# ebanalyse/ebnerd-benchmark

Hardware: AMD Instinct MI355X
Metric: training impressions/sec (higher is better)
Workload: dtype f32

## Files before the change

### ebnerd-benchmark_amd/csrc/ebn_gemm.hip

```cpp
#include <stdlib.h>

#include "ebn_common.h"
#include "ebn_finish.h"
#include "ebn_tn_finale.h"

typedef float ebn_f32x4 __attribute__((ext_vector_type(4)));
typedef int ebn_i32x4 __attribute__((ext_vector_type(4)));
__device__ ebn_f32x4 ebn_raw_buffer_load_x4(ebn_i32x4 rsrc, int voffset, int soffset, int aux) __asm("llvm.amdgcn.raw.buffer.load.v4f32");
__device__ void ebn_raw_buffer_load_lds(ebn_i32x4 rsrc, __attribute__((address_space(3))) void* lds, int size, int voffset,
                                        int soffset, int offset, int aux) __asm("llvm.amdgcn.raw.buffer.load.lds");

int ebn_gemm_direct_tn_slices(int64_t M, int64_t N, int64_t K);
int ebn_gemm_direct_tn_launch(int64_t M, int64_t N, int64_t K, float alpha, const float* A, int64_t lda, const float* B, int64_t ldb,
                              float* part, hipStream_t s);
bool ebn_gemm_direct_wanted(int32_t transA, int32_t transB, int64_t M, int64_t N, int64_t K);
int ebn_gemm_direct_launch(int32_t transB, int64_t M, int64_t N, int64_t K, float alpha, const float* A, int64_t lda, const float* B,
                           int64_t ldb, float* C, int64_t ldc, hipStream_t s);

namespace {

typedef float f32x16 __attribute__((ext_vector_type(16)));


typedef float f32x4n __attribute__((ext_vector_type(4)));
__device__ __forceinline__ float4 gload4(const __attribute__((address_space(1))) float* p) {
  const f32x4n t = *reinterpret_cast<const __attribute__((address_space(1))) f32x4n*>(p);
  return make_float4(t.x, t.y, t.z, t.w);
}
typedef ebn_i32x4 i32x4n;
__device__ __forceinline__ i32x4n make_rsrc(const float* base) {
  const unsigned long long a = reinterpret_cast<unsigned long long>(base);
  i32x4n r;
  r.x = static_cast<int>(static_cast<uint32_t>(a));
  r.y = static_cast<int>(static_cast<uint32_t>(a >> 32) & 0xFFFFu);
  r.z = -1;
  r.w = 0x00020000;
  return r;
}
__device__ __forceinline__ float4 bload4(i32x4n r, uint32_t lane_bytes, uint32_t slab_bytes) {
  const f32x4n t = ebn_raw_buffer_load_x4(r, static_cast<int>(lane_bytes), static_cast<int>(slab_bytes), 0);
  return make_float4(t.x, t.y, t.z, t.w);
}

constexpr int GEMM_WPE = 3;
constexpr int BK = 16;
constexpr int PAD = 4;
constexpr int GEMM_THREADS = 256;

template <int BMN, bool KCONTIG, bool VEC, int PADX = PAD>
struct TileLoader {
  static constexpr int VECS = BMN * BK / 4;
  static constexpr int PER_THREAD = VECS / GEMM_THREADS;
  static_assert(VECS % GEMM_THREADS == 0, "tile/thread mismatch");

  __device__ static __forceinline__ float4 load(const float* __restrict__ P, int64_t ld, int64_t mn0,
                                                int64_t k0, int64_t MN, int64_t Kdim, int v) {
    int64_t gmn, gk;
    if (KCONTIG) {
      gmn = mn0 + v / (BK / 4);
      gk = k0 + (v % (BK / 4)) * 4;
    } else {
      gk = k0 + v / (BMN / 4);
      gmn = mn0 + (v % (BMN / 4)) * 4;
    }
    const int64_t off = KCONTIG ? (gmn * ld + gk) : (gk * ld + gmn);
    if (VEC) {
      const bool valid = (gmn < MN) && (gk < Kdim);
      const float4 r = *reinterpret_cast<const float4*>(P + (valid ? off : 0));
      float4 z;
      z.x = valid ? r.x : 0.f;
      z.y = valid ? r.y : 0.f;
      z.z = valid ? r.z : 0.f;
      z.w = valid ? r.w : 0.f;
      return z;
    }
    float4 r = make_float4(0.f, 0.f, 0.f, 0.f);
    if (KCONTIG) {
      if (gmn < MN) {
        const float* p = P + off;
        if (gk + 0 < Kdim) r.x = p[0];
        if (gk + 1 < Kdim) r.y = p[1];
        if (gk + 2 < Kdim) r.z = p[2];
        if (gk + 3 < Kdim) r.w = p[3];
      }
    } else {
      if (gk < Kdim) {
        const float* p = P + off;
        if (gmn + 0 < MN) r.x = p[0];
        if (gmn + 1 < MN) r.y = p[1];
        if (gmn + 2 < MN) r.z = p[2];
        if (gmn + 3 < MN) r.w = p[3];
      }
    }
    return r;
  }

  __device__ static __forceinline__ void store(float* __restrict__ S, int v, float4 r) {
    constexpr int LD = BMN + PADX;
    if (KCONTIG) {
      const int mn = v / (BK / 4);
      const int kq = v % (BK / 4);
      *reinterpret_cast<float4*>(&S[(mn * 4 + (kq ^ ((mn >> 2) & 3))) * 4]) = r;
    } else {
      const int k = v / (BMN / 4);
      const int mq = v % (BMN / 4);
      *reinterpret_cast<float4*>(&S[k * LD + mq * 4]) = r;
    }
  }
};

struct GemmEpi {
  const float* rs;
  const float* cv;
  int64_t ldcv;
  int32_t L;
  const float* bias;
  float* colsum = nullptr;
  const float* l2w = nullptr;
  float two_lambda = 0.f;
  const int32_t* rowmap = nullptr;
  int64_t rowmap_rows = 0;
  int32_t* oob = nullptr;
#ifdef EBN_GEMM_EXP_STAGGER
  uint32_t stagger_pct = 0;
#endif
};

template <int BM, int BN, int WAVES_M, bool TA, bool TB, bool VEC, int EPI = 0>
__global__ __launch_bounds__(GEMM_THREADS, GEMM_WPE) void gemm_f32_kernel(
    int64_t M, int64_t N, int64_t K, float alpha, const float* __restrict__ A, int64_t lda,
    const float* __restrict__ B, int64_t ldb, float beta, float* __restrict__ C, int64_t ldc,
    int64_t k_per_split, float* __restrict__ Cpart, GemmEpi epi) {
  constexpr int WAVES_N = 4 / WAVES_M;
  constexpr int WTM = BM / WAVES_M;
  constexpr int WTN = BN / WAVES_N;
  constexpr int TM = WTM / 32;
  constexpr int TN = WTN / 32;
  constexpr bool GLDS_A = VEC;
  constexpr bool GLDS_B = GLDS_A;
  constexpr int PADA = GLDS_A ? 0 : PAD, PADB = GLDS_B ? 0 : PAD;
  constexpr int LDA_S = BM + PADA;
  constexpr int LDB_S = BN + PADB;
  using LA = TileLoader<BM, !TA, VEC, PADA>;
  using LB = TileLoader<BN, TB, VEC, PADB>;

  constexpr bool A_KC = !TA, B_KC = TB;
  constexpr int A_FLOATS = A_KC ? BM * BK : BK * LDA_S, B_FLOATS = B_KC ? BN * BK : BK * LDB_S;
  __shared__ __attribute__((aligned(16))) float smem[2 * (A_FLOATS + B_FLOATS)];
#define EBN_AS(b) (smem + (b) * A_FLOATS)
#define EBN_BS(b) (smem + 2 * A_FLOATS + (b) * B_FLOATS)

  const int tid = threadIdx.x;
  const int lane = tid & 63;
  const int wave = __builtin_amdgcn_readfirstlane(tid >> 6);
  const int wm = wave / WAVES_N;
  const int wn = wave % WAVES_N;
  const int64_t GX = gridDim.x, GY = gridDim.y, GZ = gridDim.z;
  const int64_t per_z = GX * GY, nwg = per_z * GZ;
  const int64_t vb = static_cast<int64_t>(blockIdx.y) * gridDim.x + blockIdx.x + per_z * blockIdx.z;
  int64_t m0 = 0, n0 = 0, kbeg = 0, kend = 0, zsplit = 0;
  int nk = 0, nk_full = 0, nk_main = 0;
// ... 148 lines not shown
  if (VEC) {                                                                             \
    const int krem__ = static_cast<int>(kend - kbeg) - (KT) * BK;                        \
    _Pragma("unroll") for (int i = 0; i < LA::PER_THREAD; ++i) {                         \
      const int v__ = tid + i * GEMM_THREADS;                                            \
      EBN_TAIL_PIECE(ra[i], arsrc, oa[i], sa, TA ? v__ / (BM / 4) : (v__ % (BK / 4)) * 4); \
    }                                                                                    \
    _Pragma("unroll") for (int i = 0; i < LB::PER_THREAD; ++i) {                         \
      const int v__ = tid + i * GEMM_THREADS;                                            \
      EBN_TAIL_PIECE(rb[i], brsrc, ob[i], sb, TB ? (v__ % (BK / 4)) * 4 : v__ / (BN / 4)); \
    }                                                                                    \
  } else {                                                                               \
    const int64_t k0__ = kbeg + static_cast<int64_t>(KT) * BK;                           \
    _Pragma("unroll") for (int i = 0; i < LA::PER_THREAD; ++i)                           \
        ra[i] = LA::load(A, lda, m0, k0__, M, kend, tid + i * GEMM_THREADS);             \
    _Pragma("unroll") for (int i = 0; i < LB::PER_THREAD; ++i)                           \
        rb[i] = LB::load(B, ldb, n0, k0__, N, kend, tid + i * GEMM_THREADS);             \
  }                                                                                      \
  } while (0)
#define EBN_STORE_PART(BUF)                                                              \
  do {                                                                                   \
    _Pragma("unroll") for (int i = 0; i < LA::PER_THREAD; ++i) LA::store(EBN_AS(BUF), tid + i * GEMM_THREADS, ra[i]); \
    _Pragma("unroll") for (int i = 0; i < LB::PER_THREAD; ++i) LB::store(EBN_BS(BUF), tid + i * GEMM_THREADS, rb[i]); \
  } while (0)

  const int kl = lane >> 5;
  const int il = lane & 31;
  {
#pragma unroll
  for (int i = 0; i < TM; ++i)
#pragma unroll
    for (int j = 0; j < TN; ++j)
#pragma unroll
      for (int r = 0; r < 16; ++r) acc[i][j][r] = 0.f;
  if (nk_main > 0) {
    EBN_FETCH_FULL(0);
    EBN_STORE_FULL(0);
    __syncthreads();
  }
#define EBN_MMA(CUR)  \
  {  \
    const float* as = A_KC ? EBN_AS((CUR)) + (wm * WTM + il) * 16 : EBN_AS((CUR)) + (4 * kl) * LDA_S + wm * WTM + il;  \
    const float* bs = B_KC ? EBN_BS((CUR)) + (wn * WTN + il) * 16 : EBN_BS((CUR)) + (4 * kl) * LDB_S + wn * WTN + il;  \
    const int sw = (il >> 2) & 3;  \
_Pragma("unroll")  \
    for (int j8 = 0; j8 < BK / 8; ++j8) {  \
      float a[TM][4], b[TN][4];  \
_Pragma("unroll")  \
      for (int i = 0; i < TM; ++i) {  \
        if (A_KC) {  \
          const float* pa__ = as + i * 32 * 16 + (((2 * j8 + kl) ^ sw) * 4);  \
          a[i][0] = pa__[0]; a[i][1] = pa__[1]; a[i][2] = pa__[2]; a[i][3] = pa__[3];  \
        } else {  \
_Pragma("unroll")  \
          for (int w = 0; w < 4; ++w) a[i][w] = as[(8 * j8 + w) * LDA_S + i * 32];  \
        }  \
      }  \
_Pragma("unroll")  \
      for (int j = 0; j < TN; ++j) {  \
        if (B_KC) {  \
          const float* pb__ = bs + j * 32 * 16 + (((2 * j8 + kl) ^ sw) * 4);  \
          b[j][0] = pb__[0]; b[j][1] = pb__[1]; b[j][2] = pb__[2]; b[j][3] = pb__[3];  \
        } else {  \
_Pragma("unroll")  \
          for (int w = 0; w < 4; ++w) b[j][w] = bs[(8 * j8 + w) * LDB_S + j * 32];  \
        }  \
      }  \
_Pragma("unroll")  \
      for (int w = 0; w < 4; ++w)  \
_Pragma("unroll")  \
        for (int i = 0; i < TM; ++i)  \
_Pragma("unroll")  \
          for (int j = 0; j < TN; ++j)  \
            acc[i][j] = __builtin_amdgcn_mfma_f32_32x32x2f32(a[i][w], b[j][w], acc[i][j], 0, 0, 0);  \
    }  \
  }
#define EBN_SLAB(CUR, KT)  \
  {  \
    const bool next__ = (KT) + 1 < nk_main;  \
    if (next__) EBN_FETCH_FULL((CUR) ^ 1);  \
    EBN_MMA(CUR)  \
    if (next__) EBN_STORE_FULL((CUR) ^ 1);  \
    __syncthreads();  \
  }
  for (int kt = 0; kt < nk_main; kt += 2) {
    EBN_SLAB(0, kt);
    if (kt + 1 < nk_main) EBN_SLAB(1, kt + 1);
  }
#undef EBN_SLAB
  if (nk_main < nk) {
    int cur = nk_main & 1;
    EBN_FETCH_PART(nk_main);
    EBN_STORE_PART(cur);
    __syncthreads();
    for (int kt = nk_main; kt < nk; ++kt) {
      if (kt + 1 < nk) EBN_FETCH_PART(kt + 1);
      EBN_MMA(cur)
      if (kt + 1 < nk) EBN_STORE_PART(cur ^ 1);
      __syncthreads();
      cur ^= 1;
    }
  }
  const int64_t em0 = m0, en0 = n0, ezs = zsplit;

  if constexpr (EPI == 1 || EPI == 2) {
    const bool split = GZ > 1;
    float* out = split ? (Cpart + ezs * M * N) : C;
    const int64_t ldo = split ? N : ldc;
    const bool read_c = !split && beta != 0.f;
#pragma unroll
    for (int i = 0; i < TM; ++i) {
#pragma unroll
      for (int j = 0; j < TN; ++j) {
        const int64_t col = en0 + wn * WTN + j * 32 + (lane & 31);
        const bool col_ok = col < N;
        const int64_t colc = col_ok ? col : N - 1;
        const int64_t row_base = em0 + wm * WTM + i * 32 + 4 * (lane >> 5);
        float add[16];
#pragma unroll
        for (int r = 0; r < 16; ++r) add[r] = 0.f;
        if (EPI == 1 && !split) {
#pragma unroll
          for (int r = 0; r < 16; ++r) {
            const int64_t row = row_base + (r & 3) + 8 * (r >> 2);
            const uint32_t rowc = static_cast<uint32_t>(row < M ? row : M - 1);
            add[r] = epi.rs[rowc] * epi.cv[static_cast<int64_t>(rowc / static_cast<uint32_t>(epi.L)) * epi.ldcv + colc];
          }
        }
        if (EPI == 2 && !split) {
          const float bv = epi.bias[colc];
#pragma unroll
          for (int r = 0; r < 16; ++r) add[r] = bv;
        }
        if (read_c) {
#pragma unroll
          for (int r = 0; r < 16; ++r) {
            const int64_t row = row_base + (r & 3) + 8 * (r >> 2);
            add[r] = fmaf(beta, out[(row < M ? row : M - 1) * ldo + colc], add[r]);
          }
        }
#pragma unroll
        for (int r = 0; r < 16; ++r) {
          const int64_t row = row_base + (r & 3) + 8 * (r >> 2);
          float v = fmaf(alpha, acc[i][j][r], add[r]);
          if (EPI == 2 && !split) v = fmaxf(v, 0.f);
          if (col_ok && row < M) out[row * ldo + col] = v;
        }
      }
    }

  } else {
    const bool split = GZ > 1;
    float* out = split ? (Cpart + ezs * M * N) : C;
    const int64_t ldo = split ? N : ldc;
#pragma unroll
    for (int i = 0; i < TM; ++i) {
#pragma unroll
      for (int j = 0; j < TN; ++j) {
        const int64_t col = en0 + wn * WTN + j * 32 + (lane & 31);
        if (col >= N) continue;
#pragma unroll
        for (int r = 0; r < 16; ++r) {
          const int64_t row = em0 + wm * WTM + i * 32 + (r & 3) + 8 * (r >> 2) + 4 * (lane >> 5);
          if (row >= M) continue;
          float v = alpha * acc[i][j][r];
          if (!split && beta != 0.f) v += beta * out[row * ldo + col];
          if (EPI == 1 && !split)
            v = fmaf(epi.rs[row], epi.cv[static_cast<int64_t>(static_cast<uint32_t>(row) / static_cast<uint32_t>(epi.L)) * epi.ldcv + col], v);
          if (EPI == 2 && !split) v = fmaxf(v + epi.bias[col], 0.f);
#if defined(EBN_GEMM_EXP_NOSTORE)
          if (v == 1.2345e38f) out[row * ldo + col] = v;
#elif defined(EBN_GEMM_EXP_NT)
          __builtin_nontemporal_store(v, &out[row * ldo + col]);
#else
          out[row * ldo + col] = v;
#endif
        }
      }
    }

  }
  }
#undef EBN_MMA
#undef EBN_FETCH_FULL
#undef EBN_FETCH_PART
#undef EBN_STORE_FULL
#undef EBN_STORE_PART
#undef EBN_TAIL_PIECE
#undef EBN_GLDS_A_DST
#undef EBN_GLDS_B_DST
#undef EBN_AS
#undef EBN_BS
#undef EBN_STORE_SLAB
}

__global__ __launch_bounds__(256) void splitk_reduce_kernel(const float* __restrict__ part, int splits,
                                                            int64_t M, int64_t N, float beta,
                                                            float* __restrict__ C, int64_t ldc, GemmEpi epi) {
  ebn_splitk_sum_body(blockIdx.x * 256u + threadIdx.x, gridDim.x * 256u, part, splits, static_cast<uint32_t>(M * N), static_cast<uint32_t>(N),
                      beta, C, ldc, epi.rs, epi.cv, epi.ldcv, epi.L, epi.bias);
}

template <int BM, int BN, int WAVES_M>
int launch_gemm(int transA, int transB, int64_t M, int64_t N, int64_t K, float alpha, const float* A,
                int64_t lda, const float* B, int64_t ldb, float beta, float* C, int64_t ldc, int vecA,
                int vecB, int splits, int64_t k_per_split, float* part, hipStream_t s, int site, GemmEpi epi) {
  dim3 grid(static_cast<unsigned>(ebn_ceil_div(N, BN)), static_cast<unsigned>(ebn_ceil_div(M, BM)),
            static_cast<unsigned>(splits));
  dim3 block(GEMM_THREADS);
#ifdef EBN_GEMM_EXP_STAGGER
  static const uint32_t stagger_pct = getenv("EBN_GEMM_STAGGER_PCT") ? static_cast<uint32_t>(atoi(getenv("EBN_GEMM_STAGGER_PCT"))) : 0u;
  epi.stagger_pct = splits == 1 ? stagger_pct : 0u;
#endif
#define EBN_GEMM_LAUNCH(TA, TB)                                                                            \
  do {                                                                                                    \
    if (vecA && vecB)                                                                                     \
      EBN_LAUNCH((gemm_f32_kernel<BM, BN, WAVES_M, TA, TB, true>), grid, block, 0, s, M, N, K, alpha, A, lda, \
                         B, ldb, beta, C, ldc, k_per_split, part, epi);                       \
    else if constexpr (BM == 64 && BN == 64)  \
      EBN_LAUNCH((gemm_f32_kernel<BM, BN, WAVES_M, TA, TB, false>), grid, block, 0, s, M, N, K, alpha, A,  \
                         lda, B, ldb, beta, C, ldc, k_per_split, part, epi);                  \
    else                                                                                                  \
      return EBN_ERR_UNSUPPORTED;                                                                         \
  } while (0)
  if (epi.rowmap != nullptr) {
    if constexpr (BM == 256)
      EBN_LAUNCH((gemm_f32_kernel<BM, BN, WAVES_M, false, false, true, 3>), grid, block, 0, s, M, N, K, alpha, A, lda, B, ldb, beta,
                         C, ldc, k_per_split, part, epi);
    else
      return EBN_ERR_UNSUPPORTED;
  } else if (epi.bias != nullptr)
    EBN_LAUNCH((gemm_f32_kernel<BM, BN, WAVES_M, false, false, true, 2>), grid, block, 0, s, M, N, K, alpha, A, lda,
                       B, ldb, beta, C, ldc, k_per_split, part, epi);
  else if (epi.rs != nullptr)
    EBN_LAUNCH((gemm_f32_kernel<BM, BN, WAVES_M, false, true, true, 1>), grid, block, 0, s, M, N, K, alpha, A, lda,
                       B, ldb, beta, C, ldc, k_per_split, part, epi);
  else if (!transA && !transB) EBN_GEMM_LAUNCH(false, false);
  else if (!transA && transB) EBN_GEMM_LAUNCH(false, true);
  else if (transA && !transB) EBN_GEMM_LAUNCH(true, false);
  else EBN_GEMM_LAUNCH(true, true);
#undef EBN_GEMM_LAUNCH
  EBN_CHECK_LAUNCH();
  return EBN_OK;
}


typedef float f32x4 __attribute__((ext_vector_type(4)));
constexpr int SBM = 32, SBN = 32;
constexpr int SBK = 128;
constexpr int SLD = SBK + 4;
constexpr int SLV = SBK + 8;
constexpr int SPT = SBM * SBK / 4 / GEMM_THREADS;

template <bool KC, bool VEC>
__device__ __forceinline__ void small_load(float4 (&r)[SPT], const float* __restrict__ P, int64_t ld, int64_t mn0, int64_t k0,
                                           int64_t MN, int64_t Kend, int tid) {
#pragma unroll
  for (int i = 0; i < SPT; ++i) {
    const int v = tid + i * GEMM_THREADS;
    if (KC) {
      int64_t mn = mn0 + v / (SBK / 4);
      mn = mn < MN ? mn : MN - 1;
      const int64_t k = k0 + (v % (SBK / 4)) * 4;
      const float* p = P + mn * ld;
      if (VEC) {
        const bool ok = k < Kend;
        const float4 t = *reinterpret_cast<const float4*>(p + (ok ? k : 0));
        r[i] = make_float4(ok ? t.x : 0.f, ok ? t.y : 0.f, ok ? t.z : 0.f, ok ? t.w : 0.f);
      } else {
        const float t0 = p[k + 0 < Kend ? k + 0 : 0], t1 = p[k + 1 < Kend ? k + 1 : 0], t2 = p[k + 2 < Kend ? k + 2 : 0],
                    t3 = p[k + 3 < Kend ? k + 3 : 0];
        r[i] = make_float4(k + 0 < Kend ? t0 : 0.f, k + 1 < Kend ? t1 : 0.f, k + 2 < Kend ? t2 : 0.f, k + 3 < Kend ? t3 : 0.f);
      }
    } else {
      const int64_t k = k0 + v / (SBM / 4);
      const bool kok = k < Kend;
      const float* p = P + (kok ? k : 0) * ld;
      const int64_t mn = mn0 + (v % (SBM / 4)) * 4;
      if (VEC) {
        const float4 t = *reinterpret_cast<const float4*>(p + (mn + 3 < MN ? mn : MN - 4));
        r[i] = make_float4(kok ? t.x : 0.f, kok ? t.y : 0.f, kok ? t.z : 0.f, kok ? t.w : 0.f);
      } else {
        const float t0 = p[mn + 0 < MN ? mn + 0 : MN - 1], t1 = p[mn + 1 < MN ? mn + 1 : MN - 1],
                    t2 = p[mn + 2 < MN ? mn + 2 : MN - 1], t3 = p[mn + 3 < MN ? mn + 3 : MN - 1];
        r[i] = make_float4(kok ? t0 : 0.f, kok ? t1 : 0.f, kok ? t2 : 0.f, kok ? t3 : 0.f);
      }
    }
  }
}

template <bool KC>
__device__ __forceinline__ void small_store(float* __restrict__ S, const float4 (&r)[SPT], int tid) {
#pragma unroll
  for (int i = 0; i < SPT; ++i) {
    const int v = tid + i * GEMM_THREADS;
    if (KC) {
      *reinterpret_cast<float4*>(&S[(v / (SBK / 4)) * SLD + (v % (SBK / 4)) * 4]) = r[i];
    } else {
      const int k = v / (SBM / 4), m4 = (v % (SBM / 4)) * 4;
      S[(m4 + 0) * SLD + k] = r[i].x;
      S[(m4 + 1) * SLD + k] = r[i].y;
      S[(m4 + 2) * SLD + k] = r[i].z;
      S[(m4 + 3) * SLD + k] = r[i].w;
    }
  }
}

template <bool TA, bool TB, bool VECA, bool VECB>
__global__ __launch_bounds__(GEMM_THREADS) void gemm_small_kernel(int64_t M, int64_t N, int64_t K, float alpha,
                                                                  const float* __restrict__ A, int64_t lda,
                                                                  const float* __restrict__ B, int64_t ldb, float beta,
                                                                  float* __restrict__ C, int64_t ldc, GemmEpi epi) {
  extern __shared__ __attribute__((aligned(16))) float smem_small[];
  const int tid = threadIdx.x, lane = tid & 63, wave = tid >> 6;
  const int wm = wave >> 1, wn = wave & 1;
  const int64_t m0 = static_cast<int64_t>(blockIdx.y) * SBM, n0 = static_cast<int64_t>(blockIdx.x) * SBN;
  const int nk = static_cast<int>((K + SBK - 1) / SBK);
  constexpr int TILE = SBM * SLD;
  f32x4 acc = {0.f, 0.f, 0.f, 0.f};
  float4 ra[SPT], rb[SPT];
  small_load<!TA, VECA>(ra, A, lda, m0, 0, M, K, tid);
  small_load<TB, VECB>(rb, B, ldb, n0, 0, N, K, tid);
  small_store<!TA>(smem_small, ra, tid);
  small_store<TB>(smem_small + TILE, rb, tid);
  __syncthreads();
  const int r16 = lane & 15, kq = lane >> 4;
  int cur = 0;
  for (int kt = 0; kt < nk; ++kt) {
    if (kt + 1 < nk) {
      small_load<!TA, VECA>(ra, A, lda, m0, static_cast<int64_t>(kt + 1) * SBK, M, K, tid);
      small_load<TB, VECB>(rb, B, ldb, n0, static_cast<int64_t>(kt + 1) * SBK, N, K, tid);
    }
    const float* ap = smem_small + cur * 2 * TILE + (wm * 16 + r16) * SLD + kq * 8;
    const float* bp = smem_small + cur * 2 * TILE + TILE + (wn * 16 + r16) * SLD + kq * 8;
    const int groups = static_cast<int>((K - static_cast<int64_t>(kt) * SBK + 31) / 32);
#pragma unroll
// ... 786 lines not shown
```

### ebnerd-benchmark_amd/csrc/ebn_gemm_direct.hip

```cpp
#include <stdlib.h>

#include "ebn_common.h"

typedef float ebn_dir_f32x4 __attribute__((ext_vector_type(4)));
typedef int ebn_dir_i32x4 __attribute__((ext_vector_type(4)));
__device__ ebn_dir_f32x4 ebn_dir_buffer_load_x4(ebn_dir_i32x4 rsrc, int voffset, int soffset, int aux) __asm("llvm.amdgcn.raw.buffer.load.v4f32");
__device__ float ebn_dir_buffer_load_x1(ebn_dir_i32x4 rsrc, int voffset, int soffset, int aux) __asm("llvm.amdgcn.raw.buffer.load.f32");

namespace {

constexpr bool INTERLEAVE = true;
typedef float f32x4 __attribute__((ext_vector_type(4)));

__device__ __forceinline__ ebn_dir_i32x4 dir_rsrc(const float* base) {
  const unsigned long long a = reinterpret_cast<unsigned long long>(base);
  ebn_dir_i32x4 r;
  r.x = static_cast<int>(static_cast<uint32_t>(a));
  r.y = static_cast<int>(static_cast<uint32_t>(a >> 32) & 0xFFFFu);
  r.z = -1;
  r.w = 0x00020000;
  return r;
}

template <int R, int NC>
struct DirFrags {
  f32x4 a[R];
  f32x4 b[NC];
};

template <int R, int NC, bool B_KC>
struct DirPlan {
  ebn_dir_i32x4 arsrc, brsrc;
  uint32_t oa[R];
  uint32_t ob[NC];
  uint32_t ldb4;
};

template <int R, int NC, bool B_KC>
__device__ __forceinline__ void dir_fetch(DirFrags<R, NC>& f, const DirPlan<R, NC, B_KC>& p, uint32_t sa, uint32_t sb) {
#pragma unroll
  for (int r = 0; r < R; ++r) f.a[r] = ebn_dir_buffer_load_x4(p.arsrc, static_cast<int>(p.oa[r]), static_cast<int>(sa), 0);
  if (B_KC) {
#pragma unroll
    for (int c = 0; c < NC; ++c) f.b[c] = ebn_dir_buffer_load_x4(p.brsrc, static_cast<int>(p.ob[c]), static_cast<int>(sb), 0);
  } else {
#pragma unroll
    for (int s = 0; s < 4; ++s)
#pragma unroll
      for (int c = 0; c < NC; ++c)
        f.b[c][s] = ebn_dir_buffer_load_x1(p.brsrc, static_cast<int>(p.ob[c]), static_cast<int>(sb + static_cast<uint32_t>(s) * p.ldb4), 0);
  }
}

template <int R, int NC, bool B_KC>
__device__ __forceinline__ void dir_fetch_tail(DirFrags<R, NC>& f, const DirPlan<R, NC, B_KC>& p, uint32_t sa, uint32_t sb, bool ok) {
  const f32x4 zero = {0.f, 0.f, 0.f, 0.f};
#pragma unroll
  for (int r = 0; r < R; ++r) {
    const f32x4 t = ebn_dir_buffer_load_x4(p.arsrc, static_cast<int>(ok ? p.oa[r] + sa : 0u), 0, 0);
    f.a[r] = ok ? t : zero;
  }
  if (B_KC) {
#pragma unroll
    for (int c = 0; c < NC; ++c) {
      const f32x4 t = ebn_dir_buffer_load_x4(p.brsrc, static_cast<int>(ok ? p.ob[c] + sb : 0u), 0, 0);
      f.b[c] = ok ? t : zero;
    }
  } else {
#pragma unroll
    for (int s = 0; s < 4; ++s)
#pragma unroll
      for (int c = 0; c < NC; ++c) {
        const float t = ebn_dir_buffer_load_x1(p.brsrc, static_cast<int>(ok ? p.ob[c] + sb + static_cast<uint32_t>(s) * p.ldb4 : 0u), 0, 0);
        f.b[c][s] = ok ? t : 0.f;
      }
  }
}

template <int R, int NC>
__device__ __forceinline__ void dir_mma(f32x4 (&acc)[R][NC], const DirFrags<R, NC>& f) {
#pragma unroll
  for (int s = 0; s < 4; ++s)
#pragma unroll
    for (int r = 0; r < R; ++r)
#pragma unroll
      for (int c = 0; c < NC; ++c) acc[r][c] = __builtin_amdgcn_mfma_f32_16x16x4f32(f.a[r][s], f.b[c][s], acc[r][c], 0, 0, 0);
}

template <int R, int NC, bool B_KC, int DEPTH>
__device__ __forceinline__ void dir_task(int64_t M, int64_t N, int64_t K, float alpha, const float* __restrict__ A, int64_t lda,
                                         const float* __restrict__ B, int64_t ldb, float* __restrict__ C, int64_t ldc, int64_t rb0,
                                         int cb0, int lane) {
  const int ln = lane & 15, kq = lane >> 4;
  const int64_t row0 = rb0 * 16;
  DirPlan<R, NC, B_KC> p;
  p.arsrc = dir_rsrc(A + row0 * lda);
  p.brsrc = dir_rsrc(B);
  p.ldb4 = static_cast<uint32_t>(ldb * 4);
#pragma unroll
  for (int r = 0; r < R; ++r) {
    int64_t row = row0 + 16 * r + ln;
    row = row < M ? row : M - 1;
    p.oa[r] = static_cast<uint32_t>(((row - row0) * lda + 4 * kq) * 4);
  }
#pragma unroll
  for (int c = 0; c < NC; ++c) {
    int64_t col = static_cast<int64_t>(cb0 + c) * 16 + ln;
    col = col < N ? col : N - 1;
    p.ob[c] = B_KC ? static_cast<uint32_t>((col * ldb + 4 * kq) * 4) : static_cast<uint32_t>((4 * kq * ldb + col) * 4);
  }
  const uint32_t step_a = 64u, step_b = B_KC ? 64u : static_cast<uint32_t>(16 * ldb * 4);

  f32x4 acc[R][NC];
#pragma unroll
  for (int r = 0; r < R; ++r)
#pragma unroll
    for (int c = 0; c < NC; ++c) acc[r][c] = f32x4{0.f, 0.f, 0.f, 0.f};

  const int nkf = static_cast<int>(K / 16);
  const int krem = static_cast<int>(K - 16 * static_cast<int64_t>(nkf));
  DirFrags<R, NC> f0, f1;
  uint32_t sa = 0, sb = 0;
  constexpr int N_LOADS = R + (B_KC ? NC : 4 * NC), N_MFMA = 4 * R * NC, PER_LOAD = (N_MFMA / N_LOADS) > 0 ? (N_MFMA / N_LOADS) : 1;
#define EBN_DIR_STEP(FL, FM)                                                   \
  do {                                                                         \
    dir_fetch(FL, p, sa, sb);                                                  \
    sa += step_a;                                                              \
    sb += step_b;                                                              \
    dir_mma(acc, FM);                                                          \
    if (INTERLEAVE) {                                                          \
      _Pragma("unroll") for (int i__ = 0; i__ < N_LOADS; ++i__) {              \
        __builtin_amdgcn_sched_group_barrier(0x008, PER_LOAD, 0);    \
        __builtin_amdgcn_sched_group_barrier(0x020, 1, 0);         \
      }                                                                        \
      __builtin_amdgcn_sched_group_barrier(0x008, N_MFMA - PER_LOAD * N_LOADS, 0); \
    }                                                                          \
    __builtin_amdgcn_sched_barrier(0);                                         \
  } while (0)
#define EBN_DIR_FETCH(F)               \
  do {                                 \
    dir_fetch(F, p, sa, sb);           \
    sa += step_a;                      \
    sb += step_b;                      \
    __builtin_amdgcn_sched_barrier(0); \
  } while (0)
#define EBN_DIR_MMA(F)                 \
  do {                                 \
    dir_mma(acc, F);                   \
    __builtin_amdgcn_sched_barrier(0); \
  } while (0)
  {
    if (nkf > 0) {
      EBN_DIR_FETCH(f0);
      int g = 0;
      for (; g + 2 < nkf; g += 2) {
        EBN_DIR_STEP(f1, f0);
        EBN_DIR_STEP(f0, f1);
      }
      if (g + 1 < nkf) {
        EBN_DIR_STEP(f1, f0);
        EBN_DIR_MMA(f1);
      } else {
        EBN_DIR_MMA(f0);
      }
    }
  }
#undef EBN_DIR_FETCH
#undef EBN_DIR_MMA
#undef EBN_DIR_STEP
  if (krem > 0) {
    dir_fetch_tail(f0, p, sa, sb, 4 * kq < krem);
    dir_mma(acc, f0);
  }

#pragma unroll
  for (int r = 0; r < R; ++r) {
#pragma unroll
    for (int c = 0; c < NC; ++c) {
      const int64_t col = static_cast<int64_t>(cb0 + c) * 16 + ln;
#pragma unroll
      for (int i = 0; i < 4; ++i) {
        const int64_t row = row0 + 16 * r + 4 * kq + i;
        if (row < M && col < N) C[row * ldc + col] = alpha * acc[r][c][i];
      }
    }
  }
}

template <int R, int CW, bool B_KC, int DEPTH>
__global__ __launch_bounds__(256, 2) void gemm_direct16_kernel(int64_t M, int64_t N, int64_t K, float alpha, const float* __restrict__ A,
                                                               int64_t lda, const float* __restrict__ B, int64_t ldb,
                                                               float* __restrict__ C, int64_t ldc, int32_t G, int32_t n_wide, int64_t n_tasks) {
  const int lane = threadIdx.x & 63;
  const int wave = __builtin_amdgcn_readfirstlane(threadIdx.x >> 6);
  const int64_t t = static_cast<int64_t>(blockIdx.x) * 4 + wave;
  if (t >= n_tasks) return;
  const int64_t rg = t / G;
  const int cg = static_cast<int>(t - rg * G);
  const int cb0 = cg < n_wide ? cg * CW : n_wide * CW + (cg - n_wide) * (CW - 1);
  if (cg < n_wide) dir_task<R, CW, B_KC, DEPTH>(M, N, K, alpha, A, lda, B, ldb, C, ldc, rg * R, cb0, lane);
  else dir_task<R, CW - 1, B_KC, DEPTH>(M, N, K, alpha, A, lda, B, ldb, C, ldc, rg * R, cb0, lane);
}

template <int R, int NC>
struct TnPlan {
  ebn_dir_i32x4 arsrc, brsrc;
  uint32_t oa[R], ob[NC];
  uint32_t lda4, ldb4;
};

template <int R, int NC>
__device__ __forceinline__ void tn_fetch(DirFrags<R, NC>& f, const TnPlan<R, NC>& p, uint32_t sa, uint32_t sb) {
#pragma unroll
  for (int s = 0; s < 4; ++s) {
#pragma unroll
    for (int r = 0; r < R; ++r)
      f.a[r][s] = ebn_dir_buffer_load_x1(p.arsrc, static_cast<int>(p.oa[r]), static_cast<int>(sa + static_cast<uint32_t>(s) * p.lda4), 0);
#pragma unroll
    for (int c = 0; c < NC; ++c)
      f.b[c][s] = ebn_dir_buffer_load_x1(p.brsrc, static_cast<int>(p.ob[c]), static_cast<int>(sb + static_cast<uint32_t>(s) * p.ldb4), 0);
  }
}

template <int R, int NC>
__device__ __forceinline__ void tn_fetch_tail(DirFrags<R, NC>& f, const TnPlan<R, NC>& p, uint32_t sa, uint32_t sb, int kq, int krem) {
#pragma unroll
  for (int s = 0; s < 4; ++s) {
    const bool ok = 4 * kq + s < krem;
#pragma unroll
    for (int r = 0; r < R; ++r) {
      const float t = ebn_dir_buffer_load_x1(p.arsrc, static_cast<int>(ok ? p.oa[r] + sa + static_cast<uint32_t>(s) * p.lda4 : 0u), 0, 0);
      f.a[r][s] = ok ? t : 0.f;
    }
#pragma unroll
    for (int c = 0; c < NC; ++c) {
      const float t = ebn_dir_buffer_load_x1(p.brsrc, static_cast<int>(ok ? p.ob[c] + sb + static_cast<uint32_t>(s) * p.ldb4 : 0u), 0, 0);
      f.b[c][s] = ok ? t : 0.f;
    }
  }
}

template <int R, int NC>
__device__ __forceinline__ void tn_task(float* red, int64_t M, int64_t N, float alpha, const float* __restrict__ A, int64_t lda,
                                        const float* __restrict__ B, int64_t ldb, float* __restrict__ out, int64_t k0, int64_t klen,
                                        int64_t rb0, int cb0, int lane, int wave) {
  const int ln = lane & 15, kq = lane >> 4;
  TnPlan<R, NC> p;
  p.arsrc = dir_rsrc(A + k0 * lda);
  p.brsrc = dir_rsrc(B + k0 * ldb);
  p.lda4 = static_cast<uint32_t>(lda * 4);
  p.ldb4 = static_cast<uint32_t>(ldb * 4);
#pragma unroll
  for (int r = 0; r < R; ++r) {
    int64_t m = (rb0 + r) * 16 + ln;
    m = m < M ? m : M - 1;
    p.oa[r] = static_cast<uint32_t>((4 * kq * lda + m) * 4);
  }
#pragma unroll
  for (int c = 0; c < NC; ++c) {
    int64_t n = static_cast<int64_t>(cb0 + c) * 16 + ln;
    n = n < N ? n : N - 1;
    p.ob[c] = static_cast<uint32_t>((4 * kq * ldb + n) * 4);
  }
  f32x4 acc[R][NC];
#pragma unroll
  for (int r = 0; r < R; ++r)
#pragma unroll
    for (int c = 0; c < NC; ++c) acc[r][c] = f32x4{0.f, 0.f, 0.f, 0.f};

  const int ng = static_cast<int>((klen + 15) / 16), krem = static_cast<int>(klen - 16 * (klen / 16));
  const int mine = ng > wave ? (ng - wave + 3) / 4 : 0;
  const bool tail_mine = krem > 0 && mine > 0 && ((ng - 1) & 3) == wave;
  const int nkf = mine - (tail_mine ? 1 : 0);
  const uint32_t step_a = 64u * p.lda4, step_b = 64u * p.ldb4;
  uint32_t sa = static_cast<uint32_t>(wave) * 16u * p.lda4, sb = static_cast<uint32_t>(wave) * 16u * p.ldb4;
  DirFrags<R, NC> f0, f1;
  constexpr int N_LOADS = 4 * (R + NC), N_MFMA = 4 * R * NC, PER_LOAD = (N_MFMA / N_LOADS) > 0 ? (N_MFMA / N_LOADS) : 1;
#define EBN_TN_FETCH(F)                \
  do {                                 \
    tn_fetch(F, p, sa, sb);            \
    sa += step_a;                      \
    sb += step_b;                      \
    __builtin_amdgcn_sched_barrier(0); \
  } while (0)
#define EBN_TN_STEP(FL, FM)                                                    \
  do {                                                                         \
    tn_fetch(FL, p, sa, sb);                                                   \
    sa += step_a;                                                              \
    sb += step_b;                                                              \
    dir_mma(acc, FM);                                                          \
    if (INTERLEAVE) {                                                          \
      _Pragma("unroll") for (int i__ = 0; i__ < N_LOADS; ++i__) {              \
        __builtin_amdgcn_sched_group_barrier(0x008, PER_LOAD, 0);              \
        __builtin_amdgcn_sched_group_barrier(0x020, 1, 0);                     \
      }                                                                        \
      __builtin_amdgcn_sched_group_barrier(0x008, N_MFMA - PER_LOAD * N_LOADS, 0); \
    }                                                                          \
    __builtin_amdgcn_sched_barrier(0);                                         \
  } while (0)
  if (nkf > 0) {
    EBN_TN_FETCH(f0);
    int g = 0;
    for (; g + 2 < nkf; g += 2) {
      EBN_TN_STEP(f1, f0);
      EBN_TN_STEP(f0, f1);
    }
    if (g + 1 < nkf) {
      EBN_TN_STEP(f1, f0);
      dir_mma(acc, f1);
    } else {
      dir_mma(acc, f0);
    }
  }
#undef EBN_TN_FETCH
#undef EBN_TN_STEP
  if (tail_mine) {
    tn_fetch_tail(f0, p, sa, sb, kq, krem);
    dir_mma(acc, f0);
  }

#pragma unroll 1
  for (int w = 1; w < 4; ++w) {
    if (wave == w) {
#pragma unroll
      for (int r = 0; r < R; ++r)
#pragma unroll
        for (int c = 0; c < NC; ++c) *reinterpret_cast<f32x4*>(red + ((r * NC + c) * 64 + lane) * 4) = acc[r][c];
    }
    __syncthreads();
    if (wave == 0) {
#pragma unroll
      for (int r = 0; r < R; ++r)
#pragma unroll
        for (int c = 0; c < NC; ++c) acc[r][c] += *reinterpret_cast<const f32x4*>(red + ((r * NC + c) * 64 + lane) * 4);
    }
    __syncthreads();
  }
  if (wave != 0) return;
#pragma unroll
  for (int r = 0; r < R; ++r) {
#pragma unroll
    for (int c = 0; c < NC; ++c) {
      const int64_t col = static_cast<int64_t>(cb0 + c) * 16 + ln;
#pragma unroll
      for (int i = 0; i < 4; ++i) {
        const int64_t row = (rb0 + r) * 16 + 4 * kq + i;
        if (row < M && col < N) out[row * N + col] = alpha * acc[r][c][i];
      }
    }
  }
}

template <int R, int CW>
__global__ __launch_bounds__(256, (R * CW >= 20) ? 1 : 2) void gemm_direct16_tn_kernel(int64_t M, int64_t N, int64_t K, float alpha, const float* __restrict__ A,
                                                                  int64_t lda, const float* __restrict__ B, int64_t ldb,
                                                                  float* __restrict__ part, int32_t G, int32_t n_wide, int32_t tiles,
                                                                  int64_t kps) {
  __shared__ __attribute__((aligned(16))) float red[R * CW * 256];
  const int lane = threadIdx.x & 63;
  const int wave = __builtin_amdgcn_readfirstlane(threadIdx.x >> 6);
  int64_t lin = blockIdx.x;
  {
    const int64_t nwg = gridDim.x, q = nwg / 8, r = nwg % 8, xcd = lin % 8, idx = lin / 8;
    lin = ((xcd < r) ? xcd * (q + 1) : r * (q + 1) + (xcd - r) * q) + idx;
  }
  const int64_t z = lin / tiles;
  const int tile = static_cast<int>(lin - z * tiles);
  const int rg = tile / G, cg = tile - rg * G;
  const int cb0 = cg < n_wide ? cg * CW : n_wide * CW + (cg - n_wide) * (CW - 1);
  const int64_t k0 = z * kps;
  const int64_t klen = (k0 + kps < K) ? kps : K - k0;
  float* out = part + z * M * N;
  if (cg < n_wide) tn_task<R, CW>(red, M, N, alpha, A, lda, B, ldb, out, k0, klen, static_cast<int64_t>(rg) * R, cb0, lane, wave);
  else tn_task<R, CW - 1>(red, M, N, alpha, A, lda, B, ldb, out, k0, klen, static_cast<int64_t>(rg) * R, cb0, lane, wave);
}

struct TnDirectPlan {
  int R, CW, G, n_wide, tiles, Z;
  int64_t kps;
};

TnDirectPlan tn_direct_plan(int64_t M, int64_t N, int64_t K) {
  const int64_t MB = ebn_ceil_div(M, 16), NB = ebn_ceil_div(N, 16);
  TnDirectPlan best{0, 0, 0, 0, 0, 0, 0};
  double best_cost = 1e300;
  static const int kR[3] = {5, 4, 3}, kC[2] = {5, 4};
  constexpr int wgs = 256;
  for (int ci = 0; ci < 2; ++ci) {
    const int64_t cw = kC[ci], G = ebn_ceil_div(NB, cw), n_wide = NB - G * (cw - 1);
    if (n_wide < 0 || n_wide > G) continue;
    for (int ri = 0; ri < 3; ++ri) {
      const int64_t tiles = ebn_ceil_div(MB, kR[ri]) * G;
      if (tiles > wgs) continue;
      int64_t Z = wgs / tiles;
      if (Z < 2) continue;
      if (Z > 64) Z = 64;
      const int64_t kps = ebn_ceil_div(ebn_ceil_div(K, Z), 64) * 64;
      Z = ebn_ceil_div(K, kps);
      if (Z < 2 || kps < 256) continue;
      const double cost = static_cast<double>(kR[ri] * (n_wide > 0 ? cw : cw - 1)) * static_cast<double>(kps / 64) * (tiles * Z > wgs ? 2.0 : 1.0);
      if (cost < best_cost) {
        best_cost = cost;
        best = TnDirectPlan{kR[ri], static_cast<int>(cw), static_cast<int>(G), static_cast<int>(n_wide), static_cast<int>(tiles), static_cast<int>(Z), kps};
      }
    }
  }
  return best;
}

struct DirectPlan {
  int R, CW, G, n_wide;
  int64_t tasks;
  double cost;
};

DirectPlan direct_plan(int64_t M, int64_t N, bool b_kc) {
  const int64_t MB = ebn_ceil_div(M, 16), NB = ebn_ceil_div(N, 16);
  DirectPlan best{0, 0, 0, 0, 0, 1e300};
  static const int kR[4] = {4, 3, 2, 1}, kC[3] = {7, 5, 4};
  for (int ci = 0; ci < 3; ++ci) {
    const int64_t cw = kC[ci], G = ebn_ceil_div(NB, cw), n_wide = NB - G * (cw - 1);
    if (n_wide < 0 || n_wide > G) continue;
    const int64_t width = n_wide > 0 ? cw : cw - 1;
    for (int ri = 0; ri < 4; ++ri) {
      if (b_kc && kR[ri] == 1) continue;
      const int64_t tasks = ebn_ceil_div(MB, kR[ri]) * G;
      const double rounds = static_cast<double>(ebn_ceil_div(tasks, 1024));
      const double cost = rounds * kR[ri] * static_cast<double>(width) * (1.0 + 0.02 * static_cast<double>(kR[ri] + width) / static_cast<double>(kR[ri] * width));
      if (cost < best.cost) best = DirectPlan{kR[ri], static_cast<int>(cw), static_cast<int>(G), static_cast<int>(n_wide), tasks, cost};
    }
  }
  return best;
}

template <int R, int CW>
int direct_launch_rc(bool b_kc, const DirectPlan& pl, int64_t M, int64_t N, int64_t K, float alpha, const float* A, int64_t lda, const float* B,
                     int64_t ldb, float* C, int64_t ldc, hipStream_t s) {
  const dim3 grid(static_cast<unsigned>(ebn_ceil_div(pl.tasks, 4))), block(256);
#define EBN_DIR_GO(KC, DP) \
  EBN_LAUNCH((gemm_direct16_kernel<R, CW, KC, DP>), grid, block, 0, s, M, N, K, alpha, A, lda, B, ldb, C, ldc, pl.G, pl.n_wide, pl.tasks)
  if constexpr (R == 1) {
    if (b_kc) return EBN_ERR_UNSUPPORTED;
    EBN_DIR_GO(false, 2);
  } else if (b_kc) EBN_DIR_GO(true, 2);
  else EBN_DIR_GO(false, 2);
#undef EBN_DIR_GO
  EBN_CHECK_LAUNCH();
  return EBN_OK;
}

}

bool ebn_gemm_direct_wanted(int32_t transA, int32_t transB, int64_t M, int64_t N, int64_t K) {
  if (transA) return false;
  if (M < 4096 || N < 48 || N > 512 || K < 32 || K > 2048 || (K % 4)) return false;
  constexpr int64_t max_b = int64_t{2} << 20;
  if (N * K * 4 > max_b) return false;
  const DirectPlan pl = direct_plan(M, N, transB != 0);
  if (pl.R == 0) return false;
  if (N * K * 4 > (int64_t{1} << 20) && M * K * 4 > (int64_t{128} << 20)) return false;
  return true;
}

int ebn_gemm_direct_launch(int32_t transB, int64_t M, int64_t N, int64_t K, float alpha, const float* A, int64_t lda, const float* B,
                           int64_t ldb, float* C, int64_t ldc, hipStream_t s) {
  if ((64 * lda + K) * 4 >= (int64_t{1} << 31) || ((transB ? N : K) * ldb + (transB ? K : N) + 16 * ldb) * 4 >= (int64_t{1} << 31)) return EBN_ERR_UNSUPPORTED;
  const DirectPlan pl = direct_plan(M, N, transB != 0);
  if (pl.R == 0 || ebn_ceil_div(pl.tasks, 4) >= (int64_t{1} << 31)) return EBN_ERR_UNSUPPORTED;
  const bool kc = transB != 0;
#define EBN_DIR_CASE(RR, CC) \
  if (pl.R == RR && pl.CW == CC) return direct_launch_rc<RR, CC>(kc, pl, M, N, K, alpha, A, lda, B, ldb, C, ldc, s)
  EBN_DIR_CASE(4, 7); EBN_DIR_CASE(3, 7); EBN_DIR_CASE(2, 7); EBN_DIR_CASE(1, 7);
  EBN_DIR_CASE(4, 5); EBN_DIR_CASE(3, 5); EBN_DIR_CASE(2, 5); EBN_DIR_CASE(1, 5);
  EBN_DIR_CASE(4, 4); EBN_DIR_CASE(3, 4); EBN_DIR_CASE(2, 4); EBN_DIR_CASE(1, 4);
#undef EBN_DIR_CASE
  return EBN_ERR_UNSUPPORTED;
}

int ebn_gemm_direct_tn_slices(int64_t M, int64_t N, int64_t K) {
  if (M < 48 || N < 48 || M > 512 || N > 1280 || K < 4096) return 0;
  return tn_direct_plan(M, N, K).Z;
}

int ebn_gemm_direct_tn_launch(int64_t M, int64_t N, int64_t K, float alpha, const float* A, int64_t lda, const float* B, int64_t ldb,
                              float* part, hipStream_t s) {
  const TnDirectPlan pl = tn_direct_plan(M, N, K);
  if (pl.Z < 2) return EBN_ERR_UNSUPPORTED;
  if ((pl.kps + 16) * (lda > ldb ? lda : ldb) * 4 >= (int64_t{1} << 31)) return EBN_ERR_UNSUPPORTED;
  const dim3 grid(static_cast<unsigned>(pl.tiles * pl.Z)), block(256);
#define EBN_TN_CASE(RR, CC)                                                                                                        \
  if (pl.R == RR && pl.CW == CC) {                                                                                                 \
// ... 10 lines not shown
```

Baseline: 25570.

## Stage GEMM epilogue tiles through LDS for coalesced 128-bit buffer stores

For full, aligned output tiles, each wave now writes its MFMA accumulators into a per-wave LDS staging tile, reads them back row-contiguously, and issues 16-byte raw buffer stores. This replaces the scattered scalar stores in the main GEMM epilogue (EPI==0, 128x64 or split 256 tiles) and in the direct and TN split-k kernels. The aim is to cut store transactions and improve write coalescing. The cost is extra LDS traffic, wave barriers, a new shared-memory allocation in the direct kernel that may lower occupancy, and a separate fast path with its own alignment and bounds checks.

```diff
diff --git a/ebnerd-benchmark_amd/csrc/ebn_gemm.hip b/ebnerd-benchmark_amd/csrc/ebn_gemm.hip
--- a/ebnerd-benchmark_amd/csrc/ebn_gemm.hip
+++ b/ebnerd-benchmark_amd/csrc/ebn_gemm.hip
@@ -7,6 +7,7 @@
 typedef float ebn_f32x4 __attribute__((ext_vector_type(4)));
 typedef int ebn_i32x4 __attribute__((ext_vector_type(4)));
 __device__ ebn_f32x4 ebn_raw_buffer_load_x4(ebn_i32x4 rsrc, int voffset, int soffset, int aux) __asm("llvm.amdgcn.raw.buffer.load.v4f32");
+__device__ void ebn_raw_buffer_store_x4(ebn_f32x4 data, ebn_i32x4 rsrc, int voffset, int soffset, int aux) __asm("llvm.amdgcn.raw.buffer.store.v4f32");
 __device__ void ebn_raw_buffer_load_lds(ebn_i32x4 rsrc, __attribute__((address_space(3))) void* lds, int size, int voffset,
                                         int soffset, int offset, int aux) __asm("llvm.amdgcn.raw.buffer.load.lds");
 
@@ -461,6 +462,57 @@
     const bool split = GZ > 1;
     float* out = split ? (Cpart + ezs * M * N) : C;
     const int64_t ldo = split ? N : ldc;
+#if !defined(EBN_GEMM_EXP_NOSTORE) && !defined(EBN_GEMM_EXP_NT)
+#define EBN_LDS_TURN()                              \
+  do {                                              \
+    __builtin_amdgcn_fence(__ATOMIC_RELEASE, "wavefront"); \
+    __builtin_amdgcn_s_waitcnt(0xc07f);             \
+    __builtin_amdgcn_wave_barrier();                \
+    __builtin_amdgcn_fence(__ATOMIC_ACQUIRE, "wavefront"); \
+    __builtin_amdgcn_sched_barrier(0);              \
+  } while (0)
+    bool fast = false;
+    if constexpr (EPI == 0) {
+      static_assert(sizeof(smem) >= 4 * 1024 * sizeof(float), "a 32 x 32 staging tile per wave");
+      constexpr bool family = BM == 128 && BN == 64;
+      fast = (family || (BM == 256 && split)) && em0 + BM <= M && en0 + BN <= N && (ldo & 3) == 0 &&
+             ldo <= (int64_t{1} << 20) &&
+             (reinterpret_cast<unsigned long long>(out) & 15ull) == 0ull && (split || beta == 0.f);
+    }
+    if (fast) {
+      float* T = smem + wave * 1024;
+      const i32x4n crsrc = make_rsrc(out + (em0 + wm * WTM) * ldo + en0 + wn * WTN);
+      const uint32_t ldo4 = static_cast<uint32_t>(ldo) * 4u;
+      const uint32_t lo = static_cast<uint32_t>(lane >> 3) * ldo4 + static_cast<uint32_t>(lane & 7) * 16u;
+      float* tw = T + (4 * kl) * 32 + il;
+      const float* tr = T + lane * 4;
+#pragma unroll
+      for (int i = 0; i < TM; ++i) {
+        f32x4n v[TN][4];
+#pragma unroll
+        for (int j = 0; j < TN; ++j) {
+#pragma unroll
+          for (int r = 0; r < 16; ++r) tw[((r & 3) + 8 * (r >> 2)) * 32] = alpha * acc[i][j][r];
+          EBN_LDS_TURN();
+#pragma unroll
+          for (int p = 0; p < 4; ++p) v[j][p] = *reinterpret_cast<const f32x4n*>(tr + p * 256);
+          EBN_LDS_TURN();
+        }
+#pragma unroll
+        for (int j = 0; j < TN; ++j)
+#pragma unroll
+          for (int p = 0; p < 4; ++p)
+            ebn_raw_buffer_store_x4(v[j][p], crsrc, static_cast<int>(lo), static_cast<int>(static_cast<uint32_t>(i * 32 + p * 8) * ldo4 + j * 128u), 0);
+        if (i + 1 < TM) {
+          __builtin_amdgcn_sched_barrier(0);
+          __builtin_amdgcn_s_waitcnt(0x0f70);
+          __builtin_amdgcn_sched_barrier(0);
+        }
+      }
+      return;
+    } else
+#endif
+    {
 #pragma unroll
     for (int i = 0; i < TM; ++i) {
 #pragma unroll
@@ -486,10 +538,12 @@
         }
       }
     }
+    }
 
   }
   }
 #undef EBN_MMA
+#undef EBN_LDS_TURN
 #undef EBN_FETCH_FULL
 #undef EBN_FETCH_PART
 #undef EBN_STORE_FULL
diff --git a/ebnerd-benchmark_amd/csrc/ebn_gemm_direct.hip b/ebnerd-benchmark_amd/csrc/ebn_gemm_direct.hip
--- a/ebnerd-benchmark_amd/csrc/ebn_gemm_direct.hip
+++ b/ebnerd-benchmark_amd/csrc/ebn_gemm_direct.hip
@@ -5,6 +5,7 @@
 typedef float ebn_dir_f32x4 __attribute__((ext_vector_type(4)));
 typedef int ebn_dir_i32x4 __attribute__((ext_vector_type(4)));
 __device__ ebn_dir_f32x4 ebn_dir_buffer_load_x4(ebn_dir_i32x4 rsrc, int voffset, int soffset, int aux) __asm("llvm.amdgcn.raw.buffer.load.v4f32");
+__device__ void ebn_dir_buffer_store_x4(ebn_dir_f32x4 data, ebn_dir_i32x4 rsrc, int voffset, int soffset, int aux) __asm("llvm.amdgcn.raw.buffer.store.v4f32");
 __device__ float ebn_dir_buffer_load_x1(ebn_dir_i32x4 rsrc, int voffset, int soffset, int aux) __asm("llvm.amdgcn.raw.buffer.load.f32");
 
 namespace {
@@ -87,10 +88,59 @@
       for (int c = 0; c < NC; ++c) acc[r][c] = __builtin_amdgcn_mfma_f32_16x16x4f32(f.a[r][s], f.b[c][s], acc[r][c], 0, 0, 0);
 }
 
+__device__ __forceinline__ void dir_lds_turn() {
+  __builtin_amdgcn_fence(__ATOMIC_RELEASE, "wavefront");
+  __builtin_amdgcn_s_waitcnt(0xc07f);
+  __builtin_amdgcn_wave_barrier();
+  __builtin_amdgcn_fence(__ATOMIC_ACQUIRE, "wavefront");
+  __builtin_amdgcn_sched_barrier(0);
+}
+
+template <int NC>
+constexpr int dir_stage_floats() { return 16 * (NC * 16 + 4); }
+
+template <int R, int NC>
+__device__ __forceinline__ void dir_store_rows(float* stage, const f32x4 (&acc)[R][NC], float alpha, float* base, int64_t ld, int lane) {
+  constexpr int LD = NC * 16 + 4, SEGS = NC * 4;
+  const int ln = lane & 15, kq = lane >> 4;
+  const ebn_dir_i32x4 crsrc = dir_rsrc(base);
+  const uint32_t ld4 = static_cast<uint32_t>(ld) * 4u;
+  float* tw = stage + (4 * kq) * LD + ln;
+  uint32_t lo[NC];
+  const float* tr[NC];
+#pragma unroll
+  for (int q = 0; q < NC; ++q) {
+    const int e = q * 64 + lane, row = e / SEGS, seg = e - row * SEGS;
+    lo[q] = static_cast<uint32_t>(row) * ld4 + static_cast<uint32_t>(seg) * 16u;
+    tr[q] = stage + row * LD + seg * 4;
+  }
+  f32x4 v[R][NC];
+#pragma unroll
+  for (int r = 0; r < R; ++r) {
+#pragma unroll
+    for (int c = 0; c < NC; ++c)
+#pragma unroll
+      for (int i = 0; i < 4; ++i) tw[i * LD + c * 16] = alpha * acc[r][c][i];
+    dir_lds_turn();
+#pragma unroll
+    for (int q = 0; q < NC; ++q) v[r][q] = *reinterpret_cast<const f32x4*>(tr[q]);
+    dir_lds_turn();
+  }
+#pragma unroll
+  for (int r = 0; r < R; ++r)
+#pragma unroll
+    for (int q = 0; q < NC; ++q)
+      ebn_dir_buffer_store_x4(v[r][q], crsrc, static_cast<int>(lo[q]), static_cast<int>(static_cast<uint32_t>(r * 16) * ld4), 0);
+}
+
+__device__ __forceinline__ bool dir_store_rows_ok(int64_t row_end, int64_t col_end, int64_t M, int64_t N, const float* base, int64_t ld) {
+  return row_end <= M && col_end <= N && (ld & 3) == 0 && ld <= (int64_t{1} << 20) && (reinterpret_cast<unsigned long long>(base) & 15ull) == 0ull;
+}
+
 template <int R, int NC, bool B_KC, int DEPTH>
 __device__ __forceinline__ void dir_task(int64_t M, int64_t N, int64_t K, float alpha, const float* __restrict__ A, int64_t lda,
                                          const float* __restrict__ B, int64_t ldb, float* __restrict__ C, int64_t ldc, int64_t rb0,
-                                         int cb0, int lane) {
+                                         int cb0, int lane, float* stage) {
   const int ln = lane & 15, kq = lane >> 4;
   const int64_t row0 = rb0 * 16;
   DirPlan<R, NC, B_KC> p;
@@ -173,6 +223,11 @@
     dir_mma(acc, f0);
   }
 
+  float* cbase = C + row0 * ldc + static_cast<int64_t>(cb0) * 16;
+  if (!B_KC && R * NC < 28 && dir_store_rows_ok(row0 + 16 * R, static_cast<int64_t>(cb0 + NC) * 16, M, N, cbase, ldc)) {
+    dir_store_rows<R, NC>(stage, acc, alpha, cbase, ldc, lane);
+    return;
+  }
 #pragma unroll
   for (int r = 0; r < R; ++r) {
 #pragma unroll
@@ -191,15 +246,17 @@
 __global__ __launch_bounds__(256, 2) void gemm_direct16_kernel(int64_t M, int64_t N, int64_t K, float alpha, const float* __restrict__ A,
                                                                int64_t lda, const float* __restrict__ B, int64_t ldb,
                                                                float* __restrict__ C, int64_t ldc, int32_t G, int32_t n_wide, int64_t n_tasks) {
+  __shared__ __attribute__((aligned(16))) float stage_all[4 * dir_stage_floats<CW>()];
   const int lane = threadIdx.x & 63;
   const int wave = __builtin_amdgcn_readfirstlane(threadIdx.x >> 6);
+  float* stage = stage_all + wave * dir_stage_floats<CW>();
   const int64_t t = static_cast<int64_t>(blockIdx.x) * 4 + wave;
   if (t >= n_tasks) return;
   const int64_t rg = t / G;
   const int cg = static_cast<int>(t - rg * G);
   const int cb0 = cg < n_wide ? cg * CW : n_wide * CW + (cg - n_wide) * (CW - 1);
-  if (cg < n_wide) dir_task<R, CW, B_KC, DEPTH>(M, N, K, alpha, A, lda, B, ldb, C, ldc, rg * R, cb0, lane);
-  else dir_task<R, CW - 1, B_KC, DEPTH>(M, N, K, alpha, A, lda, B, ldb, C, ldc, rg * R, cb0, lane);
+  if (cg < n_wide) dir_task<R, CW, B_KC, DEPTH>(M, N, K, alpha, A, lda, B, ldb, C, ldc, rg * R, cb0, lane, stage);
+  else dir_task<R, CW - 1, B_KC, DEPTH>(M, N, K, alpha, A, lda, B, ldb, C, ldc, rg * R, cb0, lane, stage);
 }
 
 template <int R, int NC>
@@ -337,6 +394,12 @@
     __syncthreads();
   }
   if (wave != 0) return;
+  static_assert(R * NC * 256 >= dir_stage_floats<NC>(), "the reduction image holds a row block's store image");
+  float* obase = out + rb0 * 16 * N + static_cast<int64_t>(cb0) * 16;
+  if (dir_store_rows_ok((rb0 + R) * 16, static_cast<int64_t>(cb0 + NC) * 16, M, N, obase, N)) {
+    dir_store_rows<R, NC>(red, acc, alpha, obase, N, lane);
+    return;
+  }
 #pragma unroll
   for (int r = 0; r < R; ++r) {
 #pragma unroll
```

After: 25700, median of 6. No clear change (+0.5%).
